# NVlabs/STEP

Measured on NVIDIA H100. Metric: clips/sec (T=32,224x224) STEP max_iter=3, higher is better.
Workload: dtype f16

## Files before the change

### step_b200/_lib.py

```python
import ctypes
import os

import torch

HERE = os.path.dirname(os.path.abspath(__file__))
LIB_PATH = os.path.join(HERE, "libstep_b200.so")

F32, F16 = 0, 1
EXT_NONE, EXT_PREDICT, EXT_EXTRAPOLATE, EXT_MEAN = 0, 1, 2, 3
A_AUTO, A_LINEAR, A_BOX, A_IM2COL, A_HALO, A_BEST, A_SIMT = 0, 1, 2, 3, 4, 5, 9

_lib = None

c_int, c_float, c_void_p, c_size_t = ctypes.c_int, ctypes.c_float, ctypes.c_void_p, ctypes.c_size_t


class ConvParams(ctypes.Structure):
    _fields_ = [(n, c_int) for n in
                ("dtype", "N", "T", "H", "W", "Cin", "in_ld", "Cout", "out_ld", "out_coff", "KT", "KH", "KW",
                 "ST", "SH", "SW", "PT", "PH", "PW", "OT", "OH", "OW", "relu", "w_ld")] + \
               [("x", c_void_p), ("w", c_void_p), ("scale", c_void_p), ("shift", c_void_p),
                ("residual", c_void_p), ("res_ld", c_int), ("res_coff", c_int), ("y", c_void_p),
                ("a_mode", c_int), ("n_splits", c_int), ("split", c_int * 2), ("y_extra", c_void_p * 2),
                ("ld_extra", c_int * 2), ("coff_extra", c_int * 2), ("zero_cin_last_kt", c_int)]
# ... 37 lines not shown
        "step_clip_to_s2d_f16": ([P, I, I, I, I, I, P, I, S], c_int),
        "step_nhwc_to_nchw_f32": ([P, I, I, I, I, I, P, S], c_int),
        "step_nchw_to_nhwc": ([P, I, I, I, P, I, I, S], c_int),
        "step_conv3d_fwd": ([ctypes.POINTER(ConvParams), S], c_int),
        "step_maxpool3d_fwd": ([P, I] + [I] * 21 + [P, I, S], c_int),
        "step_mean_mid": ([P, I, I, I, I, I, I, P, I, S], c_int),
        "step_mean_mid_strided": ([P, I, I, I, I, I, I, ctypes.c_longlong, P, I, S], c_int),
        "step_linear_small_n_workspace_bytes": ([I, I, I], c_size_t),
        "step_linear_small_n": ([P, I, I, I, I, P, P, I, P, I, I, I, P, P, c_size_t, S], c_int),
        "step_head_regress": ([P, I, I, I, I, I, P, P, I, I, I, I, P, P, P, P, c_size_t, S], c_int),
        "step_bottleneck_exit_f16": ([P, ctypes.c_longlong, P, P, ctypes.c_longlong, P, P, I, P, ctypes.c_longlong, P, ctypes.c_longlong,
                                     ctypes.c_longlong, I, I, I, S], c_int),
        "step_head_losses_f32": ([P, P, P, P, P, P, I, I, I, I, I, Fl, Fl, P, P, P, P, P, P, P, P, P, S], c_int),
        "step_cls_loss_f32": ([P, P, I, I, P, P, P, S], c_int),
        "step_roi_align_bwd_nhwc": ([P, I, I, P, I, Fl, I, I, I, I, I, I, I, P, I, S], c_int),
        "step_roi_align_bwd_slice_workspace_bytes": ([I, I, I, I, I, I], c_size_t),
        "step_roi_align_bwd_slice_nhwc": ([P, I, I, P, I, Fl, I, I, I, I, I, I, I, I, I, I, P, I, P, c_size_t, S], c_int),
        "step_ctx_grad_reduce_f32": ([P, I, P, I, I, I, I, I, I, P, S], c_int),
        "step_linear_small_n_bwd": ([P, I, I, I, I, P, P, I, P, I, P, P, S], c_int),
        "step_conv1x1_wgrad_workspace_bytes": ([I, I, I], c_size_t),
        "step_conv1x1_wgrad_f16": ([P, I, P, I, I, I, I, Fl, P, I, I, P, c_size_t, S], c_int),
        "step_conv_wgrad_workspace_bytes": ([I, I, I, I], c_size_t),
        "step_conv_wgrad_f16": ([P, I, P, I, I, I, I, I, I, I, I, I, I, I, I, I, Fl, P, I, I, P, c_size_t, S], c_int),
        "step_act_bwd_f16": ([P, I, P, I, P, I, ctypes.c_longlong, I, P, I, P, I, S], c_int),
        "step_colsum_f16": ([P, I, ctypes.c_longlong, I, Fl, P, P, S], c_int),
        "step_mean_mid_bwd": ([P, I, I, I, I, Fl, P, I, S], c_int),
        "step_f32_accum_f16": ([P, ctypes.c_longlong, I, Fl, P, I, S], c_int),
        "step_maxpool3d_bwd_f16": ([P, I, P, I] + [I] * 20 + [P, I, P, S], c_int),
        "step_multi_tensor_chunk": ([], c_int),
        "step_multi_tensor_nonfinite_f32": ([P, I, P, I, P, S], c_int),
        "step_multi_tensor_adam_f32": ([P, I, P, I, S], c_int),
        "step_multi_tensor_sgd_f32": ([P, I, P, I, S], c_int),
        "step_debug_tma_tile": ([ctypes.POINTER(ConvParams), I, I, I, I, I, P, P, P, S], c_int),
    }
    for name, (argtypes, restype) in sigs.items():
        fn = getattr(lib, name)
        fn.argtypes = argtypes
        fn.restype = restype
    return sigs


def lib():
    global _lib
    if _lib is None:
        if not os.path.exists(LIB_PATH):
            raise RuntimeError("step_b200: %s not found -- run `python -m step_b200.build` (there is no "
                               "CPU / PyTorch fallback for the hot path)" % LIB_PATH)
        l = ctypes.CDLL(LIB_PATH)
        _declare(l)
        _lib = l
    return _lib


def exported_symbols():
    return sorted(_declare(lib()).keys())


def check(rc):
    if rc != 0:
        raise RuntimeError("step_b200 [%d]: %s" % (rc, lib().step_last_error().decode("utf-8", "replace")))


def stream(device=None):
    return c_void_p(torch.cuda.current_stream(device).cuda_stream)


# ... 35 lines not shown
```

### step_b200/csrc/conv_umma.cu

```cuda
#include <cuda.h>
#include <stdlib.h>
#include <string.h>

#include "common.cuh"
#include "umma_ptx.cuh"

namespace step {

enum { A_LINEAR = 1, A_BOX = 2, A_IM2COL = 3 };

constexpr int kBM = 128;
constexpr int kMaxBN = 256;
constexpr int kStages = 8;
constexpr int kThreads = 384;
constexpr int kConsumers = 256;
constexpr int kBookBytes = 2 * kStages * 8 + 2 * kMaxBN * 4;
constexpr int kProducerRegs = 40, kConsumerRegs = 232;

#define STEP_CONV_TILES(X)                                                                                         \
  X(64, 32) X(64, 64) X(64, 128) X(64, 144) X(64, 152) X(64, 176) X(64, 192) X(64, 208) X(64, 224) X(64, 256)      \
  X(32, 64) X(32, 128) X(32, 144) X(32, 152) X(32, 160) X(32, 208) X(32, 224)                                      \
  X(16, 64)

__host__ __device__ constexpr int staging_pitch(int BN) { return ((BN / 8 + 1) | 1) * 16; }

struct ConvGeom {
  int mode;
  int taps, KT, KH, KW, PT, PH, PW;
  int kblocks_per_tap;
  int BN, n_tiles;
  int n_stages;
  int n_splits, split[2], ld_extra[2], coff_extra[2];
  __half* y_extra[2];
  int Cout, out_ld, out_coff, res_ld, res_coff, relu;
  int OT, OH, OW, Nimg;
  long long M;
  int bw, bh, bt, tiles_w, tiles_h, tiles_t;
  int a_bytes;
};

__device__ __forceinline__ long long tile_row_pixel(const ConvGeom& g, int m_tile, int row) {
  if (g.mode == A_BOX) {
    int r = m_tile;
    const int bw0 = (r % g.tiles_w) * g.bw; r /= g.tiles_w;
    const int bh0 = (r % g.tiles_h) * g.bh; r /= g.tiles_h;
    const int bt0 = (r % g.tiles_t) * g.bt; const int bn = r / g.tiles_t;
    const int dw = row % g.bw, rr = row / g.bw;
    const int dh = rr % g.bh, dt = rr / g.bh;
    const int ow = bw0 + dw, oh = bh0 + dh, ot = bt0 + dt;
    if (dt < g.bt && ow < g.OW && oh < g.OH && ot < g.OT) return (((long long)bn * g.OT + ot) * g.OH + oh) * g.OW + ow;
    return -1;
  }
  const long long m = (long long)m_tile * kBM + row;
  return m < g.M ? m : -1;
}

template <int BK, int BN>
__global__ void __launch_bounds__(kThreads, 1)
conv_umma_kernel(const __grid_constant__ CUtensorMap map_a, const __grid_constant__ CUtensorMap map_b, ConvGeom g,
                 const float* __restrict__ scale, const float* __restrict__ shift, const __half* __restrict__ residual,
                 __half* __restrict__ y) {
  static_assert(BN % 8 == 0 && BN <= kMaxBN, "wgmma N is a multiple of 8, at most 256");
  constexpr bool kRealloc = BN > 128;
  constexpr int kABytes = kBM * BK * 2;
  constexpr int kBBytes = BN * BK * 2;
  extern __shared__ __align__(1024) uint8_t smem_raw[];
  uint64_t* full_bar = (uint64_t*)smem_raw;
  uint64_t* empty_bar = full_bar + kStages;
  float* s_scale = (float*)(empty_bar + kStages);
  float* s_shift = s_scale + kMaxBN;
  uint8_t* smem = (uint8_t*)(((uintptr_t)smem_raw + kBookBytes + 1023) & ~(uintptr_t)1023);
  uint8_t* sA = smem;
  uint8_t* sB = smem + g.n_stages * kABytes;

  const int warp = threadIdx.x >> 5, lane = threadIdx.x & 31;
  const int m_tile = blockIdx.x / g.n_tiles, n_tile = blockIdx.x - m_tile * g.n_tiles;
  const int n0 = n_tile * BN;
  const int num_kb = g.taps * g.kblocks_per_tap;

  if (threadIdx.x == 0) {
    asm volatile("prefetch.tensormap [%0];" ::"l"(&map_a) : "memory");
    asm volatile("prefetch.tensormap [%0];" ::"l"(&map_b) : "memory");
    for (int s = 0; s < kStages; ++s) { mbar_init(&full_bar[s], 1); mbar_init(&empty_bar[s], 2); }
    fence_barrier_init();
  }
  if (threadIdx.x < 128) {
    for (int i = threadIdx.x; i < BN; i += 128) {
      const int c = n0 + i;
      s_scale[i] = (scale && c < g.Cout) ? scale[c] : 1.0f;
      s_shift[i] = (shift && c < g.Cout) ? shift[c] : 0.0f;
    }
  }
  __syncthreads();
  pdl_wait();
  pdl_launch_dependents();

  if (warp < 4) {
    if constexpr (kRealloc) setmaxnreg_dec<kProducerRegs>();
    if (warp == 0 && elect_one()) {
      long long m0 = (long long)m_tile * kBM;
      int bn = 0, bt0 = 0, bh0 = 0, bw0 = 0;
      if (g.mode == A_BOX) {
        int r = m_tile;
        bw0 = (r % g.tiles_w) * g.bw; r /= g.tiles_w;
        bh0 = (r % g.tiles_h) * g.bh; r /= g.tiles_h;
        bt0 = (r % g.tiles_t) * g.bt; bn = r / g.tiles_t;
      }
      int iw = 0, ih = 0, it = 0, in_ = 0;
      if (g.mode == A_IM2COL) {
        long long r = m0;
        iw = (int)(r % g.OW); r /= g.OW;
        ih = (int)(r % g.OH); r /= g.OH;
        it = (int)(r % g.OT); in_ = (int)(r / g.OT);
        iw -= g.PW; ih -= g.PH; it -= g.PT;
      }
      const uint32_t tx_bytes = (uint32_t)(g.a_bytes + kBBytes);
      int stage = 0; uint32_t phase = 0;
      int kw = 0, kh = 0, kt = 0;
      for (int tap = 0; tap < g.taps; ++tap) {
        for (int kc = 0; kc < g.kblocks_per_tap; ++kc) {
          mbar_wait(&empty_bar[stage], phase ^ 1);
          mbar_expect_tx(&full_bar[stage], tx_bytes);
          const int c0 = kc * BK;
          uint8_t* a_dst = sA + stage * kABytes;
          if (g.mode == A_LINEAR) {
            tma_load_2d(&map_a, &full_bar[stage], a_dst, c0, (int)m0);
          } else if (g.mode == A_BOX) {
            tma_load_5d(&map_a, &full_bar[stage], a_dst, c0, bw0 + kw - g.PW, bh0 + kh - g.PH, bt0 + kt - g.PT, bn);
          } else {
            tma_load_im2col_5d(&map_a, &full_bar[stage], a_dst, c0, iw, ih, it, in_, (uint16_t)kw, (uint16_t)kh, (uint16_t)kt);
          }
          tma_load_3d(&map_b, &full_bar[stage], sB + stage * kBBytes, c0, tap, n0);
          if (++stage == g.n_stages) { stage = 0; phase ^= 1; }
        }
        if (++kw == g.KW) { kw = 0; if (++kh == g.KH) { kh = 0; ++kt; } }
      }
    }
  } else {
    if constexpr (kRealloc) setmaxnreg_inc<kConsumerRegs>();
    const int wg = (warp >> 2) - 1;
    const int ct = threadIdx.x - 128;
    const uint64_t hi = desc_hi_kmajor<BK>();
    const uint64_t a_lo0 = desc_lo(sA + wg * 64 * BK * 2), b_lo0 = desc_lo(sB);
    float acc[BN / 2];
#pragma unroll
    for (int i = 0; i < BN / 2; ++i) acc[i] = 0.0f;
    int stage = 0, prev = -1; uint32_t phase = 0;
    for (int kb = 0; kb < num_kb; ++kb) {
      mbar_wait(&full_bar[stage], phase);
      const uint64_t a_lo = a_lo0 + (uint64_t)(stage * (kABytes >> 4)), b_lo = b_lo0 + (uint64_t)(stage * (kBBytes >> 4));
      wg_fence();
#pragma unroll
      for (int k = 0; k < BK / 16; ++k)
        wgmma_f16<BN>(acc, hi | (a_lo + 2 * k), hi | (b_lo + 2 * k), 1u);
      wg_commit();
      wg_wait<1>();
      if (prev >= 0 && ct % 128 == 0) mbar_arrive(&empty_bar[prev]);
      prev = stage;
      if (++stage == g.n_stages) { stage = 0; phase ^= 1; }
    }
    wg_wait<0>();
    named_sync(1, kConsumers);
    constexpr int pitch = staging_pitch(BN);
    const int wrow = wg * 64 + (warp & 3) * 16 + (lane >> 2);
#pragma unroll
    for (int i = 0; i < 2; ++i) {
      const int row = wrow + 8 * i;
      const long long pix = residual ? tile_row_pixel(g, m_tile, row) : -1;
      const __half* rrow = pix >= 0 ? residual + (size_t)pix * g.res_ld + g.res_coff + n0 : nullptr;
      uint8_t* srow = smem + (size_t)row * pitch;
#pragma unroll
      for (int j = 0; j < BN / 8; ++j) {
        const int col = 8 * j + 2 * (lane & 3);
        float f0 = fmaf(acc[4 * j + 2 * i], s_scale[col], s_shift[col]);
        float f1 = fmaf(acc[4 * j + 2 * i + 1], s_scale[col + 1], s_shift[col + 1]);
        if (rrow && n0 + col < g.Cout) {
          const float2 rf = __half22float2(*reinterpret_cast<const __half2*>(rrow + col));
          f0 += rf.x; f1 += rf.y;
        }
        if (g.relu) { f0 = fmaxf(f0, 0.0f); f1 = fmaxf(f1, 0.0f); }
        *reinterpret_cast<__half2*>(srow + col * 2) = __floats2half2_rn(f0, f1);
      }
    }
    named_sync(1, kConsumers);
    constexpr int cpr = BN / 8;
    for (int i = ct; i < kBM * cpr; i += kConsumers) {
      const int rr = i / cpr, ch = i - rr * cpr;
      const int col = n0 + ch * 8;
      if (col >= g.Cout) continue;
      const long long rp = tile_row_pixel(g, m_tile, rr);
      if (rp < 0) continue;
      const uint4 val = *reinterpret_cast<const uint4*>(smem + (size_t)rr * pitch + ch * 16);
      __half* dst = y + (size_t)rp * g.out_ld + g.out_coff + col;
      if (g.n_splits > 0 && col >= g.split[0]) {
        const int d = (g.n_splits > 1 && col >= g.split[1]) ? 1 : 0;
        dst = g.y_extra[d] + (size_t)rp * g.ld_extra[d] + g.coff_extra[d] + (col - g.split[d]);
      }
      *reinterpret_cast<uint4*>(dst) = val;
    }
  }
}

template <int BK>
__global__ void __launch_bounds__(32) tma_dump_kernel(const __grid_constant__ CUtensorMap map_a, ConvGeom g, int m_tile,
                                                      int kt, int kh, int kw, int c0, uint8_t* __restrict__ out) {
  constexpr int kABytes = kBM * BK * 2;
  extern __shared__ __align__(1024) uint8_t smem_raw[];
  uint8_t* smem = (uint8_t*)(((uintptr_t)smem_raw + 1023) & ~(uintptr_t)1023);
  __shared__ uint64_t bar;
  for (int i = threadIdx.x; i < kABytes / 4; i += 32) ((uint32_t*)smem)[i] = 0xFFFFFFFFu;
  if (threadIdx.x == 0) { mbar_init(&bar, 1); fence_barrier_init(); }
  fence_proxy_async();
  __syncwarp();
  if (threadIdx.x == 0) {
    long long m0 = (long long)m_tile * kBM;
    mbar_expect_tx(&bar, (uint32_t)g.a_bytes);
    if (g.mode == A_LINEAR) {
      tma_load_2d(&map_a, &bar, smem, c0, (int)m0);
    } else if (g.mode == A_BOX) {
      int r = m_tile;
      int bw0 = (r % g.tiles_w) * g.bw; r /= g.tiles_w;
      int bh0 = (r % g.tiles_h) * g.bh; r /= g.tiles_h;
      int bt0 = (r % g.tiles_t) * g.bt; int bn = r / g.tiles_t;
      tma_load_5d(&map_a, &bar, smem, c0, bw0 + kw - g.PW, bh0 + kh - g.PH, bt0 + kt - g.PT, bn);
    } else {
      long long r = m0;
      int iw = (int)(r % g.OW); r /= g.OW;
      int ih = (int)(r % g.OH); r /= g.OH;
      int it = (int)(r % g.OT); int in_ = (int)(r / g.OT);
      tma_load_im2col_5d(&map_a, &bar, smem, c0, iw - g.PW, ih - g.PH, it - g.PT, in_, (uint16_t)kw, (uint16_t)kh, (uint16_t)kt);
    }
// ... 158 lines not shown
                             (cuuint64_t)p->H * p->W * p->in_ld * 2, (cuuint64_t)p->T * p->H * p->W * p->in_ld * 2};
    if (mode == A_BOX) {
      pick_box(p->OW, p->OH, p->OT, &g.bw, &g.bh, &g.bt);
      g.tiles_w = (p->OW + g.bw - 1) / g.bw; g.tiles_h = (p->OH + g.bh - 1) / g.bh; g.tiles_t = (p->OT + g.bt - 1) / g.bt;
      cuuint32_t box[5] = {(cuuint32_t)BK, (cuuint32_t)g.bw, (cuuint32_t)g.bh, (cuuint32_t)g.bt, 1};
      cr = g_encode_tiled(&pl->map_a, CU_TENSOR_MAP_DATA_TYPE_FLOAT16, 5, (void*)p->x, dims, strides, box, ones,
                          CU_TENSOR_MAP_INTERLEAVE_NONE, swizzle_for(BK), CU_TENSOR_MAP_L2_PROMOTION_L2_128B,
                          CU_TENSOR_MAP_FLOAT_OOB_FILL_NONE);
      m_tiles = (long long)p->N * g.tiles_t * g.tiles_h * g.tiles_w;
      g.a_bytes = g.bw * g.bh * g.bt * BK * 2;
    } else {
      const int ph_t = p->OT - p->T + p->KT - 1 - p->PT, ph_h = p->OH - p->H + p->KH - 1 - p->PH,
                ph_w = p->OW - p->W + p->KW - 1 - p->PW;
      int lower[3] = {-p->PW, -p->PH, -p->PT};
      int upper[3] = {ph_w - (p->KW - 1), ph_h - (p->KH - 1), ph_t - (p->KT - 1)};
      for (int i = 0; i < 3; ++i)
        STEP_CHECK_ARG(lower[i] >= -16 && lower[i] <= 15 && upper[i] >= -16 && upper[i] <= 15, "conv3d(f16): im2col corner range");
      cr = g_encode_im2col(&pl->map_a, CU_TENSOR_MAP_DATA_TYPE_FLOAT16, 5, (void*)p->x, dims, strides, lower, upper,
                           (cuuint32_t)BK, (cuuint32_t)kBM, ones, CU_TENSOR_MAP_INTERLEAVE_NONE, swizzle_for(BK),
                           CU_TENSOR_MAP_L2_PROMOTION_L2_128B, CU_TENSOR_MAP_FLOAT_OOB_FILL_NONE);
      int drv = 0;
      cudaDriverGetVersion(&drv);
      if (cr == CUDA_SUCCESS && drv <= 13010 &&
          (size_t)p->N * p->T * p->H * p->W * p->in_ld * 2 < 131072)
        reinterpret_cast<uint64_t*>(&pl->map_a)[1] &= ~(1ULL << 21);
      m_tiles = (g.M + kBM - 1) / kBM;
      g.a_bytes = kBM * BK * 2;
    }
  }
  if (cr != CUDA_SUCCESS) return fail(STEP_E_DRIVER, "conv3d(f16): tensor map (A, mode %d) encode failed: CUresult %d", mode, (int)cr);
  {
    cuuint64_t dims[3] = {(cuuint64_t)p->Cin, (cuuint64_t)taps, (cuuint64_t)p->Cout};
    cuuint64_t strides[2] = {(cuuint64_t)p->w_ld * 2, (cuuint64_t)taps * p->w_ld * 2};
    cuuint32_t box[3] = {(cuuint32_t)BK, 1, (cuuint32_t)g.BN};
    cr = g_encode_tiled(&pl->map_b, CU_TENSOR_MAP_DATA_TYPE_FLOAT16, 3, (void*)p->w, dims, strides, box, ones,
                        CU_TENSOR_MAP_INTERLEAVE_NONE, swizzle_for(BK), CU_TENSOR_MAP_L2_PROMOTION_L2_256B,
                        CU_TENSOR_MAP_FLOAT_OOB_FILL_NONE);
    if (cr != CUDA_SUCCESS) return fail(STEP_E_DRIVER, "conv3d(f16): tensor map (B) encode failed: CUresult %d", (int)cr);
  }
  STEP_CHECK_ARG(m_tiles * g.n_tiles < (1LL << 31), "conv3d(f16): grid too large");
  pl->grid = dim3((unsigned)(m_tiles * g.n_tiles));
  const long per_stage = (long)kBM * BK * 2 + (long)g.BN * BK * 2;
  const long fixed = kBookBytes + 1024;
  const long out_tile = (long)kBM * staging_pitch(g.BN);
  int st = (int)((113L * 1024 - fixed) / per_stage);
  if (st > kStages) st = kStages;
  bool two = false;
  if (st >= 4) {
    const long area = st * per_stage;
    if (int rc = two_ctas_fit(pl->tile, (size_t)(fixed + (area > out_tile ? area : out_tile)), &two)) return rc;
  }
  if (!two) st = (int)((227L * 1024 - fixed) / per_stage);
  g.n_stages = st > kStages ? kStages : st;
  STEP_CHECK_ARG(g.n_stages >= 2, "conv3d(f16): tile does not fit shared memory");
  const long stage_area = g.n_stages * per_stage;
  pl->smem_bytes = (size_t)(fixed + (stage_area > out_tile ? stage_area : out_tile));
  return 0;
}

int conv3d_umma_launch(const step_conv_params* p, step_stream_t stream) {
  ConvPlan pl;
  if (int rc = build_plan(p, &pl)) return rc;
  const ConvTile& t = kTiles[pl.tile];
  if (first_use_on_device(g_attr_seen[pl.tile])) {
    cudaError_t e = cudaFuncSetAttribute(t.kernel, cudaFuncAttributeMaxDynamicSharedMemorySize, 227 * 1024);
    if (e != cudaSuccess) return fail((int)e, "conv3d(f16): smem attribute: %s", cudaGetErrorString(e));
  }
  cudaStream_t s = cu(stream);
  cudaLaunchConfig_t cfg = {};
  cudaLaunchAttribute attr[1];
  cfg.gridDim = pl.grid; cfg.blockDim = dim3(kThreads); cfg.dynamicSmemBytes = pl.smem_bytes; cfg.stream = s;
  if (pdl_enabled()) {
    attr[0].id = cudaLaunchAttributeProgrammaticStreamSerialization;
    attr[0].val.programmaticStreamSerializationAllowed = 1;
    cfg.attrs = attr; cfg.numAttrs = 1;
  }
  cudaError_t le = cudaLaunchKernelEx(&cfg, t.kernel, pl.map_a, pl.map_b, pl.g, p->scale, p->shift,
                                      (const __half*)p->residual, (__half*)p->y);
  if (le != cudaSuccess) { cudaGetLastError(); return fail((int)le, "conv_umma_kernel launch: %s", cudaGetErrorString(le)); }
  STEP_LAUNCH_CHECK("conv_umma_kernel");
  return 0;
}

}

using namespace step;

extern "C" int step_debug_tma_tile(const step_conv_params* p, int m_tile, int kt, int kh, int kw, int c0, void* out,
                                   int* bk_out, int* box_out , step_stream_t stream) {
  ConvPlan pl;
  if (int rc = build_plan(p, &pl)) return rc;
  if (bk_out) *bk_out = pl.BK;
  if (box_out) { box_out[0] = pl.g.bw; box_out[1] = pl.g.bh; box_out[2] = pl.g.bt; }
  size_t smem = 1024 + (size_t)kBM * pl.BK * 2;
  if (pl.BK == 64) tma_dump_kernel<64><<<1, 32, smem, cu(stream)>>>(pl.map_a, pl.g, m_tile, kt, kh, kw, c0, (uint8_t*)out);
  else if (pl.BK == 32) tma_dump_kernel<32><<<1, 32, smem, cu(stream)>>>(pl.map_a, pl.g, m_tile, kt, kh, kw, c0, (uint8_t*)out);
  else tma_dump_kernel<16><<<1, 32, smem, cu(stream)>>>(pl.map_a, pl.g, m_tile, kt, kh, kw, c0, (uint8_t*)out);
  STEP_LAUNCH_CHECK("tma_dump_kernel");
  return 0;
}
```

### step_b200/csrc/umma_ptx.cuh

```cuda
#pragma once
#include <cuda.h>
#include <cuda_fp16.h>
#include <stdint.h>

namespace step {

__device__ __forceinline__ uint32_t smem_u32(const void* p) { return (uint32_t)__cvta_generic_to_shared(p); }

__device__ __forceinline__ void mbar_init(uint64_t* bar, uint32_t count) {
  asm volatile("mbarrier.init.shared::cta.b64 [%0], %1;" ::"r"(smem_u32(bar)), "r"(count));
}
__device__ __forceinline__ void mbar_expect_tx(uint64_t* bar, uint32_t bytes) {
  asm volatile("mbarrier.arrive.expect_tx.shared::cta.b64 _, [%0], %1;" ::"r"(smem_u32(bar)), "r"(bytes) : "memory");
}
__device__ __forceinline__ void mbar_arrive(uint64_t* bar) {
  asm volatile("mbarrier.arrive.shared::cta.b64 _, [%0];" ::"r"(smem_u32(bar)) : "memory");
}
__device__ __forceinline__ void mbar_wait(uint64_t* bar, uint32_t parity) {
  asm volatile(
      "{\n\t.reg .pred p;\n\t"
      "WAIT_LOOP:\n\t"
      "mbarrier.try_wait.parity.shared::cta.b64 p, [%0], %1;\n\t"
      "@p bra.uni WAIT_DONE;\n\t"
      "bra.uni WAIT_LOOP;\n\t"
// ... 22 lines not shown
               ::"r"(smem_u32(dst)), "l"(map), "r"(smem_u32(bar)), "r"(c), "r"(w), "r"(h), "r"(d), "r"(n), "h"(ow), "h"(oh), "h"(od) : "memory");
}
__device__ __forceinline__ void tma_store_2d(const CUtensorMap* map, const void* src, int c0, int c1) {
  asm volatile("cp.async.bulk.tensor.2d.global.shared::cta.bulk_group [%0, {%2, %3}], [%1];"
               ::"l"(map), "r"(smem_u32(src)), "r"(c0), "r"(c1) : "memory");
}
__device__ __forceinline__ void bulk_commit() { asm volatile("cp.async.bulk.commit_group;" ::: "memory"); }
template <int N>
__device__ __forceinline__ void bulk_wait_read() { asm volatile("cp.async.bulk.wait_group.read %0;" ::"n"(N) : "memory"); }

template <int BK>
__device__ __forceinline__ uint64_t desc_hi_kmajor() {
  constexpr uint64_t sw = BK == 64 ? 1 : (BK == 32 ? 2 : 3);
  return (1ULL << 16) | ((uint64_t)((8 * BK * 2) >> 4) << 32) | (sw << 62);
}
__device__ __forceinline__ uint64_t desc_lo(const void* p) { return (uint64_t)((smem_u32(p) & 0x3FFFF) >> 4); }

__device__ __forceinline__ void wg_fence() { asm volatile("wgmma.fence.sync.aligned;" ::: "memory"); }
__device__ __forceinline__ void wg_commit() { asm volatile("wgmma.commit_group.sync.aligned;" ::: "memory"); }
template <int N>
__device__ __forceinline__ void wg_wait() { asm volatile("wgmma.wait_group.sync.aligned %0;" ::"n"(N) : "memory"); }

template <int N>
__device__ __forceinline__ void wgmma_f16(float* d, uint64_t da, uint64_t db, uint32_t accumulate);

#define STEP_D4(i) "+f"(d[4 * (i)]), "+f"(d[4 * (i) + 1]), "+f"(d[4 * (i) + 2]), "+f"(d[4 * (i) + 3])
#define STEP_WGMMA_F16(N, IA, IB, IC, REGS, ...)                                                                        \
  template <>                                                                                                          \
  __device__ __forceinline__ void wgmma_f16<N>(float* d, uint64_t da, uint64_t db, uint32_t accumulate) {              \
    asm volatile("{\n\t.reg .pred p;\n\tsetp.ne.b32 p, %" #IC ", 0;\n\t"                                              \
                 "wgmma.mma_async.sync.aligned.m64n" #N "k16.f32.f16.f16 {" REGS "}, %" #IA ", %" #IB ", p, 1, 1, 0, 0;\n\t}" \
                 : __VA_ARGS__ : "l"(da), "l"(db), "r"(accumulate));                                                    \
  }
STEP_WGMMA_F16(32, 16, 17, 18,
               "%0, %1, %2, %3, %4, %5, %6, %7, %8, %9, %10, %11, %12, %13, %14, %15",
               STEP_D4(0), STEP_D4(1), STEP_D4(2), STEP_D4(3))
STEP_WGMMA_F16(64, 32, 33, 34,
               "%0, %1, %2, %3, %4, %5, %6, %7, %8, %9, %10, %11, %12, %13, %14, %15, %16, %17, %18, %19, %20, %21, %22, "
               "%23, %24, %25, %26, %27, %28, %29, %30, %31",
               STEP_D4(0), STEP_D4(1), STEP_D4(2), STEP_D4(3), STEP_D4(4), STEP_D4(5), STEP_D4(6), STEP_D4(7))
STEP_WGMMA_F16(128, 64, 65, 66,
               "%0, %1, %2, %3, %4, %5, %6, %7, %8, %9, %10, %11, %12, %13, %14, %15, %16, %17, %18, %19, %20, %21, %22, "
               "%23, %24, %25, %26, %27, %28, %29, %30, %31, %32, %33, %34, %35, %36, %37, %38, %39, %40, %41, %42, %43, "
               "%44, %45, %46, %47, %48, %49, %50, %51, %52, %53, %54, %55, %56, %57, %58, %59, %60, %61, %62, %63",
               STEP_D4(0), STEP_D4(1), STEP_D4(2), STEP_D4(3), STEP_D4(4), STEP_D4(5), STEP_D4(6), STEP_D4(7),
               STEP_D4(8), STEP_D4(9), STEP_D4(10), STEP_D4(11), STEP_D4(12), STEP_D4(13), STEP_D4(14), STEP_D4(15))
STEP_WGMMA_F16(144, 72, 73, 74,
               "%0, %1, %2, %3, %4, %5, %6, %7, %8, %9, %10, %11, %12, %13, %14, %15, %16, %17, %18, %19, %20, %21, %22, "
               "%23, %24, %25, %26, %27, %28, %29, %30, %31, %32, %33, %34, %35, %36, %37, %38, %39, %40, %41, %42, %43, "
               "%44, %45, %46, %47, %48, %49, %50, %51, %52, %53, %54, %55, %56, %57, %58, %59, %60, %61, %62, %63, %64, "
               "%65, %66, %67, %68, %69, %70, %71",
               STEP_D4(0), STEP_D4(1), STEP_D4(2), STEP_D4(3), STEP_D4(4), STEP_D4(5), STEP_D4(6), STEP_D4(7),
               STEP_D4(8), STEP_D4(9), STEP_D4(10), STEP_D4(11), STEP_D4(12), STEP_D4(13), STEP_D4(14), STEP_D4(15),
               STEP_D4(16), STEP_D4(17))
STEP_WGMMA_F16(152, 76, 77, 78,
               "%0, %1, %2, %3, %4, %5, %6, %7, %8, %9, %10, %11, %12, %13, %14, %15, %16, %17, %18, %19, %20, %21, %22, "
               "%23, %24, %25, %26, %27, %28, %29, %30, %31, %32, %33, %34, %35, %36, %37, %38, %39, %40, %41, %42, %43, "
               "%44, %45, %46, %47, %48, %49, %50, %51, %52, %53, %54, %55, %56, %57, %58, %59, %60, %61, %62, %63, %64, "
               "%65, %66, %67, %68, %69, %70, %71, %72, %73, %74, %75",
               STEP_D4(0), STEP_D4(1), STEP_D4(2), STEP_D4(3), STEP_D4(4), STEP_D4(5), STEP_D4(6), STEP_D4(7),
               STEP_D4(8), STEP_D4(9), STEP_D4(10), STEP_D4(11), STEP_D4(12), STEP_D4(13), STEP_D4(14), STEP_D4(15),
               STEP_D4(16), STEP_D4(17), STEP_D4(18))
STEP_WGMMA_F16(160, 80, 81, 82,
               "%0, %1, %2, %3, %4, %5, %6, %7, %8, %9, %10, %11, %12, %13, %14, %15, %16, %17, %18, %19, %20, %21, %22, "
               "%23, %24, %25, %26, %27, %28, %29, %30, %31, %32, %33, %34, %35, %36, %37, %38, %39, %40, %41, %42, %43, "
               "%44, %45, %46, %47, %48, %49, %50, %51, %52, %53, %54, %55, %56, %57, %58, %59, %60, %61, %62, %63, %64, "
               "%65, %66, %67, %68, %69, %70, %71, %72, %73, %74, %75, %76, %77, %78, %79",
               STEP_D4(0), STEP_D4(1), STEP_D4(2), STEP_D4(3), STEP_D4(4), STEP_D4(5), STEP_D4(6), STEP_D4(7),
               STEP_D4(8), STEP_D4(9), STEP_D4(10), STEP_D4(11), STEP_D4(12), STEP_D4(13), STEP_D4(14), STEP_D4(15),
               STEP_D4(16), STEP_D4(17), STEP_D4(18), STEP_D4(19))
STEP_WGMMA_F16(176, 88, 89, 90,
               "%0, %1, %2, %3, %4, %5, %6, %7, %8, %9, %10, %11, %12, %13, %14, %15, %16, %17, %18, %19, %20, %21, %22, "
               "%23, %24, %25, %26, %27, %28, %29, %30, %31, %32, %33, %34, %35, %36, %37, %38, %39, %40, %41, %42, %43, "
// ... 96 lines not shown
```

Before: 1099.

## Make wgmma conv kernel persistent with half-width tail tiles and per-group epilogue

Turns the wgmma conv kernel into a persistent kernel that loops over work units with grid capped at SM slots. To cut wave-quantization tail waste, the remainder tiles are split into two half-N units using narrower wgmma shapes, and B is loaded in two half boxes. The epilogue now runs per warpgroup through a dedicated chunked staging buffer with per-group scale/shift, so each group syncs independently and smem is no longer aliased with pipeline stages. This costs extra shared memory, which may reduce pipeline stages, and adds more template code and register pressure. It also adds a debug plan query entry point.

Measured after the change: 1112 (median of 6 runs). +1.1%, better.

```diff
diff --git a/step_b200/_lib.py b/step_b200/_lib.py
--- a/step_b200/_lib.py
+++ b/step_b200/_lib.py
@@ -93,6 +93,7 @@
         "step_multi_tensor_adam_f32": ([P, I, P, I, S], c_int),
         "step_multi_tensor_sgd_f32": ([P, I, P, I, S], c_int),
         "step_debug_tma_tile": ([ctypes.POINTER(ConvParams), I, I, I, I, I, P, P, P, S], c_int),
+        "step_debug_conv_plan": ([ctypes.POINTER(ConvParams), P], c_int),
     }
     for name, (argtypes, restype) in sigs.items():
         fn = getattr(lib, name)
diff --git a/step_b200/csrc/conv_umma.cu b/step_b200/csrc/conv_umma.cu
--- a/step_b200/csrc/conv_umma.cu
+++ b/step_b200/csrc/conv_umma.cu
@@ -13,8 +13,7 @@
 constexpr int kMaxBN = 256;
 constexpr int kStages = 8;
 constexpr int kThreads = 384;
-constexpr int kConsumers = 256;
-constexpr int kBookBytes = 2 * kStages * 8 + 2 * kMaxBN * 4;
+constexpr int kBookBytes = 2 * kStages * 8 + 2 * 2 * kMaxBN * 4;
 constexpr int kProducerRegs = 40, kConsumerRegs = 232;
 
 #define STEP_CONV_TILES(X)                                                                                         \
@@ -22,7 +21,11 @@
   X(32, 64) X(32, 128) X(32, 144) X(32, 152) X(32, 160) X(32, 208) X(32, 224)                                      \
   X(16, 64)
 
-__host__ __device__ constexpr int staging_pitch(int BN) { return ((BN / 8 + 1) | 1) * 16; }
+__host__ __device__ constexpr int staging_pitch(int cols) { return ((cols / 8 + 1) | 1) * 16; }
+constexpr int kChunk = 64;
+constexpr int kGroupStaging = 64 * staging_pitch(kChunk);
+constexpr int kStagingBytes = 2 * kGroupStaging;
+__host__ __device__ constexpr bool halves_ok(int BN) { return BN % 16 == 0; }
 
 struct ConvGeom {
   int mode;
@@ -30,6 +33,7 @@
   int kblocks_per_tap;
   int BN, n_tiles;
   int n_stages;
+  int units, full_units;
   int n_splits, split[2], ld_extra[2], coff_extra[2];
   __half* y_extra[2];
   int Cout, out_ld, out_coff, res_ld, res_coff, relu;
@@ -55,27 +59,58 @@
   return m < g.M ? m : -1;
 }
 
+template <int BN>
+__device__ __forceinline__ void unit_tile(const ConvGeom& g, int u, int* m_tile, int* n0, bool* half) {
+  int t = u, h = 0;
+  *half = u >= g.full_units;
+  if (*half) { t = g.full_units + ((u - g.full_units) >> 1); h = (u - g.full_units) & 1; }
+  *m_tile = t / g.n_tiles;
+  *n0 = (t - *m_tile * g.n_tiles) * BN + h * (BN / 2);
+}
+
+template <int BK, int BN, int N>
+__device__ __forceinline__ void mma_unit(float* acc, uint64_t hi, uint64_t a_lo0, uint64_t b_lo0, int num_kb, int n_stages,
+                                         uint64_t* full_bar, uint64_t* empty_bar, bool leader, int& stage, uint32_t& phase) {
+  constexpr int kABytes = kBM * BK * 2;
+  constexpr int kBBytes = BN * BK * 2;
+  int prev = -1;
+  for (int kb = 0; kb < num_kb; ++kb) {
+    mbar_wait(&full_bar[stage], phase);
+    const uint64_t a_lo = a_lo0 + (uint64_t)(stage * (kABytes >> 4)), b_lo = b_lo0 + (uint64_t)(stage * (kBBytes >> 4));
+    wg_fence();
+#pragma unroll
+    for (int k = 0; k < BK / 16; ++k)
+      wgmma_f16<N>(acc, hi | (a_lo + 2 * k), hi | (b_lo + 2 * k), 1u);
+    wg_commit();
+    wg_wait<1>();
+    if (prev >= 0 && leader) mbar_arrive(&empty_bar[prev]);
+    prev = stage;
+    if (++stage == n_stages) { stage = 0; phase ^= 1; }
+  }
+  wg_wait<0>();
+  if (leader) mbar_arrive(&empty_bar[prev]);
+}
+
 template <int BK, int BN>
-__global__ void __launch_bounds__(kThreads, 1)
+__global__ void __launch_bounds__(kThreads, BN <= 64 ? 2 : 1)
 conv_umma_kernel(const __grid_constant__ CUtensorMap map_a, const __grid_constant__ CUtensorMap map_b, ConvGeom g,
                  const float* __restrict__ scale, const float* __restrict__ shift, const __half* __restrict__ residual,
                  __half* __restrict__ y) {
   static_assert(BN % 8 == 0 && BN <= kMaxBN, "wgmma N is a multiple of 8, at most 256");
   constexpr bool kRealloc = BN > 128;
+  constexpr bool kHalves = halves_ok(BN);
   constexpr int kABytes = kBM * BK * 2;
   constexpr int kBBytes = BN * BK * 2;
   extern __shared__ __align__(1024) uint8_t smem_raw[];
   uint64_t* full_bar = (uint64_t*)smem_raw;
   uint64_t* empty_bar = full_bar + kStages;
-  float* s_scale = (float*)(empty_bar + kStages);
-  float* s_shift = s_scale + kMaxBN;
+  float* epi_const = (float*)(empty_bar + kStages);
   uint8_t* smem = (uint8_t*)(((uintptr_t)smem_raw + kBookBytes + 1023) & ~(uintptr_t)1023);
   uint8_t* sA = smem;
   uint8_t* sB = smem + g.n_stages * kABytes;
+  uint8_t* staging = sB + g.n_stages * kBBytes;
 
   const int warp = threadIdx.x >> 5, lane = threadIdx.x & 31;
-  const int m_tile = blockIdx.x / g.n_tiles, n_tile = blockIdx.x - m_tile * g.n_tiles;
-  const int n0 = n_tile * BN;
   const int num_kb = g.taps * g.kblocks_per_tap;
 
   if (threadIdx.x == 0) {
@@ -84,13 +119,6 @@
     for (int s = 0; s < kStages; ++s) { mbar_init(&full_bar[s], 1); mbar_init(&empty_bar[s], 2); }
     fence_barrier_init();
   }
-  if (threadIdx.x < 128) {
-    for (int i = threadIdx.x; i < BN; i += 128) {
-      const int c = n0 + i;
-      s_scale[i] = (scale && c < g.Cout) ? scale[c] : 1.0f;
-      s_shift[i] = (shift && c < g.Cout) ? shift[c] : 0.0f;
-    }
-  }
   __syncthreads();
   pdl_wait();
   pdl_launch_dependents();
@@ -98,105 +126,129 @@
   if (warp < 4) {
     if constexpr (kRealloc) setmaxnreg_dec<kProducerRegs>();
     if (warp == 0 && elect_one()) {
-      long long m0 = (long long)m_tile * kBM;
-      int bn = 0, bt0 = 0, bh0 = 0, bw0 = 0;
-      if (g.mode == A_BOX) {
-        int r = m_tile;
-        bw0 = (r % g.tiles_w) * g.bw; r /= g.tiles_w;
-        bh0 = (r % g.tiles_h) * g.bh; r /= g.tiles_h;
-        bt0 = (r % g.tiles_t) * g.bt; bn = r / g.tiles_t;
-      }
-      int iw = 0, ih = 0, it = 0, in_ = 0;
-      if (g.mode == A_IM2COL) {
-        long long r = m0;
-        iw = (int)(r % g.OW); r /= g.OW;
-        ih = (int)(r % g.OH); r /= g.OH;
-        it = (int)(r % g.OT); in_ = (int)(r / g.OT);
-        iw -= g.PW; ih -= g.PH; it -= g.PT;
-      }
-      const uint32_t tx_bytes = (uint32_t)(g.a_bytes + kBBytes);
       int stage = 0; uint32_t phase = 0;
-      int kw = 0, kh = 0, kt = 0;
-      for (int tap = 0; tap < g.taps; ++tap) {
-        for (int kc = 0; kc < g.kblocks_per_tap; ++kc) {
-          mbar_wait(&empty_bar[stage], phase ^ 1);
-          mbar_expect_tx(&full_bar[stage], tx_bytes);
-          const int c0 = kc * BK;
-          uint8_t* a_dst = sA + stage * kABytes;
-          if (g.mode == A_LINEAR) {
-            tma_load_2d(&map_a, &full_bar[stage], a_dst, c0, (int)m0);
-          } else if (g.mode == A_BOX) {
-            tma_load_5d(&map_a, &full_bar[stage], a_dst, c0, bw0 + kw - g.PW, bh0 + kh - g.PH, bt0 + kt - g.PT, bn);
-          } else {
-            tma_load_im2col_5d(&map_a, &full_bar[stage], a_dst, c0, iw, ih, it, in_, (uint16_t)kw, (uint16_t)kh, (uint16_t)kt);
+      for (int u = blockIdx.x; u < g.units; u += gridDim.x) {
+        int m_tile, n0; bool half;
+        unit_tile<BN>(g, u, &m_tile, &n0, &half);
+        const long long m0 = (long long)m_tile * kBM;
+        int bn = 0, bt0 = 0, bh0 = 0, bw0 = 0;
+        if (g.mode == A_BOX) {
+          int r = m_tile;
+          bw0 = (r % g.tiles_w) * g.bw; r /= g.tiles_w;
+          bh0 = (r % g.tiles_h) * g.bh; r /= g.tiles_h;
+          bt0 = (r % g.tiles_t) * g.bt; bn = r / g.tiles_t;
+        }
+        int iw = 0, ih = 0, it = 0, in_ = 0;
+        if (g.mode == A_IM2COL) {
+          long long r = m0;
+          iw = (int)(r % g.OW); r /= g.OW;
+          ih = (int)(r % g.OH); r /= g.OH;
+          it = (int)(r % g.OT); in_ = (int)(r / g.OT);
+          iw -= g.PW; ih -= g.PH; it -= g.PT;
+        }
+        const uint32_t tx_bytes = (uint32_t)(g.a_bytes + (half ? kBBytes / 2 : kBBytes));
+        int kw = 0, kh = 0, kt = 0;
+        for (int tap = 0; tap < g.taps; ++tap) {
+          for (int kc = 0; kc < g.kblocks_per_tap; ++kc) {
+            mbar_wait(&empty_bar[stage], phase ^ 1);
+            mbar_expect_tx(&full_bar[stage], tx_bytes);
+            const int c0 = kc * BK;
+            uint8_t* a_dst = sA + stage * kABytes;
+            if (g.mode == A_LINEAR) {
+              tma_load_2d(&map_a, &full_bar[stage], a_dst, c0, (int)m0);
+            } else if (g.mode == A_BOX) {
+              tma_load_5d(&map_a, &full_bar[stage], a_dst, c0, bw0 + kw - g.PW, bh0 + kh - g.PH, bt0 + kt - g.PT, bn);
+            } else {
+              tma_load_im2col_5d(&map_a, &full_bar[stage], a_dst, c0, iw, ih, it, in_, (uint16_t)kw, (uint16_t)kh, (uint16_t)kt);
+            }
+            uint8_t* b_dst = sB + stage * kBBytes;
+            tma_load_3d(&map_b, &full_bar[stage], b_dst, c0, tap, n0);
+            if (kHalves && !half) tma_load_3d(&map_b, &full_bar[stage], b_dst + kBBytes / 2, c0, tap, n0 + BN / 2);
+            if (++stage == g.n_stages) { stage = 0; phase ^= 1; }
           }
-          tma_load_3d(&map_b, &full_bar[stage], sB + stage * kBBytes, c0, tap, n0);
-          if (++stage == g.n_stages) { stage = 0; phase ^= 1; }
+          if (++kw == g.KW) { kw = 0; if (++kh == g.KH) { kh = 0; ++kt; } }
         }
-        if (++kw == g.KW) { kw = 0; if (++kh == g.KH) { kh = 0; ++kt; } }
       }
     }
   } else {
     if constexpr (kRealloc) setmaxnreg_inc<kConsumerRegs>();
     const int wg = (warp >> 2) - 1;
-    const int ct = threadIdx.x - 128;
+    const bool leader = (threadIdx.x & 127) == 0;
     const uint64_t hi = desc_hi_kmajor<BK>();
     const uint64_t a_lo0 = desc_lo(sA + wg * 64 * BK * 2), b_lo0 = desc_lo(sB);
+    constexpr int pitch = staging_pitch(kChunk);
+    uint8_t* wstage = staging + wg * kGroupStaging;
+    float* s_scale = epi_const + wg * 2 * kMaxBN;
+    float* s_shift = s_scale + kMaxBN;
+    const int wt = threadIdx.x & 127;
+    const int lrow = (warp & 3) * 16 + (lane >> 2);
+    const int q = lane & 3;
     float acc[BN / 2];
-#pragma unroll
-    for (int i = 0; i < BN / 2; ++i) acc[i] = 0.0f;
-    int stage = 0, prev = -1; uint32_t phase = 0;
-    for (int kb = 0; kb < num_kb; ++kb) {
-      mbar_wait(&full_bar[stage], phase);
-      const uint64_t a_lo = a_lo0 + (uint64_t)(stage * (kABytes >> 4)), b_lo = b_lo0 + (uint64_t)(stage * (kBBytes >> 4));
-      wg_fence();
-#pragma unroll
-      for (int k = 0; k < BK / 16; ++k)
-        wgmma_f16<BN>(acc, hi | (a_lo + 2 * k), hi | (b_lo + 2 * k), 1u);
-      wg_commit();
-      wg_wait<1>();
-      if (prev >= 0 && ct % 128 == 0) mbar_arrive(&empty_bar[prev]);
-      prev = stage;
-      if (++stage == g.n_stages) { stage = 0; phase ^= 1; }
-    }
-    wg_wait<0>();
-    named_sync(1, kConsumers);
-    constexpr int pitch = staging_pitch(BN);
-    const int wrow = wg * 64 + (warp & 3) * 16 + (lane >> 2);
-#pragma unroll
-    for (int i = 0; i < 2; ++i) {
-      const int row = wrow + 8 * i;
-      const long long pix = residual ? tile_row_pixel(g, m_tile, row) : -1;
-      const __half* rrow = pix >= 0 ? residual + (size_t)pix * g.res_ld + g.res_coff + n0 : nullptr;
-      uint8_t* srow = smem + (size_t)row * pitch;
-#pragma unroll
-      for (int j = 0; j < BN / 8; ++j) {
-        const int col = 8 * j + 2 * (lane & 3);
-        float f0 = fmaf(acc[4 * j + 2 * i], s_scale[col], s_shift[col]);
-        float f1 = fmaf(acc[4 * j + 2 * i + 1], s_scale[col + 1], s_shift[col + 1]);
-        if (rrow && n0 + col < g.Cout) {
-          const float2 rf = __half22float2(*reinterpret_cast<const __half2*>(rrow + col));
-          f0 += rf.x; f1 += rf.y;
+    int stage = 0; uint32_t phase = 0;
+    for (int u = blockIdx.x; u < g.units; u += gridDim.x) {
+      int m_tile, n0; bool half;
+      unit_tile<BN>(g, u, &m_tile, &n0, &half);
+      const int ncols = half ? BN / 2 : BN;
+      for (int i = wt; i < ncols; i += 128) {
+        const int c = n0 + i;
+        s_scale[i] = (scale && c < g.Cout) ? scale[c] : 1.0f;
+        s_shift[i] = (shift && c < g.Cout) ? shift[c] : 0.0f;
+      }
+#pragma unroll
+      for (int i = 0; i < BN / 2; ++i) acc[i] = 0.0f;
+      if constexpr (kHalves) {
+        if (half) mma_unit<BK, BN, BN / 2>(acc, hi, a_lo0, b_lo0, num_kb, g.n_stages, full_bar, empty_bar, leader, stage, phase);
+        else mma_unit<BK, BN, BN>(acc, hi, a_lo0, b_lo0, num_kb, g.n_stages, full_bar, empty_bar, leader, stage, phase);
+      } else {
+        mma_unit<BK, BN, BN>(acc, hi, a_lo0, b_lo0, num_kb, g.n_stages, full_bar, empty_bar, leader, stage, phase);
+      }
+      const __half* rrow[2];
+#pragma unroll
+      for (int i = 0; i < 2; ++i) {
+        const long long pix = residual ? tile_row_pixel(g, m_tile, wg * 64 + lrow + 8 * i) : -1;
+        rrow[i] = pix >= 0 ? residual + (size_t)pix * g.res_ld + g.res_coff + n0 : nullptr;
+      }
+      long long opix[4];
+#pragma unroll
+      for (int k = 0; k < 4; ++k) opix[k] = tile_row_pixel(g, m_tile, wg * 64 + (wt >> 3) + 16 * k);
+      named_sync(1 + wg, 128);
+#pragma unroll
+      for (int c = 0; c < (BN + kChunk - 1) / kChunk; ++c) {
+        if (c * kChunk >= ncols) break;
+#pragma unroll
+        for (int jj = 0; jj < kChunk / 8; ++jj) {
+          const int j = c * (kChunk / 8) + jj;
+          if (j >= BN / 8 || 8 * j >= ncols) break;
+          const int col = 8 * j + 2 * q;
+#pragma unroll
+          for (int i = 0; i < 2; ++i) {
+            float f0 = fmaf(acc[4 * j + 2 * i], s_scale[col], s_shift[col]);
+            float f1 = fmaf(acc[4 * j + 2 * i + 1], s_scale[col + 1], s_shift[col + 1]);
+            if (rrow[i] && n0 + col < g.Cout) {
+              const float2 rf = __half22float2(*reinterpret_cast<const __half2*>(rrow[i] + col));
+              f0 += rf.x; f1 += rf.y;
+            }
+            if (g.relu) { f0 = fmaxf(f0, 0.0f); f1 = fmaxf(f1, 0.0f); }
+            *reinterpret_cast<__half2*>(wstage + (lrow + 8 * i) * pitch + (col - c * kChunk) * 2) = __floats2half2_rn(f0, f1);
+          }
         }
-        if (g.relu) { f0 = fmaxf(f0, 0.0f); f1 = fmaxf(f1, 0.0f); }
-        *reinterpret_cast<__half2*>(srow + col * 2) = __floats2half2_rn(f0, f1);
+        named_sync(1 + wg, 128);
+        const int ccol = c * kChunk + 8 * (wt & 7), col = n0 + ccol;
+        if (ccol < ncols && col < g.Cout) {
+#pragma unroll
+          for (int k = 0; k < 4; ++k) {
+            if (opix[k] < 0) continue;
+            const uint4 val = *reinterpret_cast<const uint4*>(wstage + ((wt >> 3) + 16 * k) * pitch + (wt & 7) * 16);
+            __half* dst = y + (size_t)opix[k] * g.out_ld + g.out_coff + col;
+            if (g.n_splits > 0 && col >= g.split[0]) {
+              const int d = (g.n_splits > 1 && col >= g.split[1]) ? 1 : 0;
+              dst = g.y_extra[d] + (size_t)opix[k] * g.ld_extra[d] + g.coff_extra[d] + (col - g.split[d]);
+            }
+            *reinterpret_cast<uint4*>(dst) = val;
+          }
+        }
+        named_sync(1 + wg, 128);
       }
-    }
-    named_sync(1, kConsumers);
-    constexpr int cpr = BN / 8;
-    for (int i = ct; i < kBM * cpr; i += kConsumers) {
-      const int rr = i / cpr, ch = i - rr * cpr;
-      const int col = n0 + ch * 8;
-      if (col >= g.Cout) continue;
-      const long long rp = tile_row_pixel(g, m_tile, rr);
-      if (rp < 0) continue;
-      const uint4 val = *reinterpret_cast<const uint4*>(smem + (size_t)rr * pitch + ch * 16);
-      __half* dst = y + (size_t)rp * g.out_ld + g.out_coff + col;
-      if (g.n_splits > 0 && col >= g.split[0]) {
-        const int d = (g.n_splits > 1 && col >= g.split[1]) ? 1 : 0;
-        dst = g.y_extra[d] + (size_t)rp * g.ld_extra[d] + g.coff_extra[d] + (col - g.split[d]);
-      }
-      *reinterpret_cast<uint4*>(dst) = val;
     }
   }
 }
@@ -421,29 +473,35 @@
   {
     cuuint64_t dims[3] = {(cuuint64_t)p->Cin, (cuuint64_t)taps, (cuuint64_t)p->Cout};
     cuuint64_t strides[2] = {(cuuint64_t)p->w_ld * 2, (cuuint64_t)taps * p->w_ld * 2};
-    cuuint32_t box[3] = {(cuuint32_t)BK, 1, (cuuint32_t)g.BN};
+    cuuint32_t box[3] = {(cuuint32_t)BK, 1, (cuuint32_t)(halves_ok(g.BN) ? g.BN / 2 : g.BN)};
     cr = g_encode_tiled(&pl->map_b, CU_TENSOR_MAP_DATA_TYPE_FLOAT16, 3, (void*)p->w, dims, strides, box, ones,
                         CU_TENSOR_MAP_INTERLEAVE_NONE, swizzle_for(BK), CU_TENSOR_MAP_L2_PROMOTION_L2_256B,
                         CU_TENSOR_MAP_FLOAT_OOB_FILL_NONE);
     if (cr != CUDA_SUCCESS) return fail(STEP_E_DRIVER, "conv3d(f16): tensor map (B) encode failed: CUresult %d", (int)cr);
   }
-  STEP_CHECK_ARG(m_tiles * g.n_tiles < (1LL << 31), "conv3d(f16): grid too large");
-  pl->grid = dim3((unsigned)(m_tiles * g.n_tiles));
+  const long long tiles = m_tiles * g.n_tiles;
+  STEP_CHECK_ARG(2 * tiles < (1LL << 31), "conv3d(f16): grid too large");
   const long per_stage = (long)kBM * BK * 2 + (long)g.BN * BK * 2;
-  const long fixed = kBookBytes + 1024;
-  const long out_tile = (long)kBM * staging_pitch(g.BN);
+  const long fixed = kBookBytes + 1024 + kStagingBytes;
   int st = (int)((113L * 1024 - fixed) / per_stage);
   if (st > kStages) st = kStages;
   bool two = false;
-  if (st >= 4) {
-    const long area = st * per_stage;
-    if (int rc = two_ctas_fit(pl->tile, (size_t)(fixed + (area > out_tile ? area : out_tile)), &two)) return rc;
-  }
+  if (st >= 4)
+    if (int rc = two_ctas_fit(pl->tile, (size_t)(fixed + st * per_stage), &two)) return rc;
   if (!two) st = (int)((227L * 1024 - fixed) / per_stage);
   g.n_stages = st > kStages ? kStages : st;
   STEP_CHECK_ARG(g.n_stages >= 2, "conv3d(f16): tile does not fit shared memory");
-  const long stage_area = g.n_stages * per_stage;
-  pl->smem_bytes = (size_t)(fixed + (stage_area > out_tile ? stage_area : out_tile));
+  pl->smem_bytes = (size_t)(fixed + g.n_stages * per_stage);
+  int dev = 0, sms = 0;
+  cudaError_t e = cudaGetDevice(&dev);
+  if (e == cudaSuccess) e = cudaDeviceGetAttribute(&sms, cudaDevAttrMultiProcessorCount, dev);
+  if (e != cudaSuccess) { cudaGetLastError(); return fail((int)e, "conv3d(f16): SM count: %s", cudaGetErrorString(e)); }
+  const long long slots = (long long)sms * (two ? 2 : 1);
+  const long long rem = tiles % slots;
+  const long long split = (halves_ok(g.BN) && 2 * rem <= slots) ? rem : 0;
+  g.full_units = (int)(tiles - split);
+  g.units = (int)(tiles + split);
+  pl->grid = dim3((unsigned)(g.units < slots ? g.units : slots));
   return 0;
 }
 
@@ -488,3 +546,11 @@
   STEP_LAUNCH_CHECK("tma_dump_kernel");
   return 0;
 }
+
+extern "C" int step_debug_conv_plan(const step_conv_params* p, int* out ) {
+  ConvPlan pl;
+  if (int rc = build_plan(p, &pl)) return rc;
+  const int v[6] = {pl.BK, pl.g.BN, pl.g.n_stages, (int)pl.grid.x, pl.g.units, pl.g.full_units};
+  for (int i = 0; i < 6; ++i) out[i] = v[i];
+  return 0;
+}
diff --git a/step_b200/csrc/umma_ptx.cuh b/step_b200/csrc/umma_ptx.cuh
--- a/step_b200/csrc/umma_ptx.cuh
+++ b/step_b200/csrc/umma_ptx.cuh
@@ -78,6 +78,9 @@
                  "wgmma.mma_async.sync.aligned.m64n" #N "k16.f32.f16.f16 {" REGS "}, %" #IA ", %" #IB ", p, 1, 1, 0, 0;\n\t}" \
                  : __VA_ARGS__ : "l"(da), "l"(db), "r"(accumulate));                                                    \
   }
+STEP_WGMMA_F16(16, 8, 9, 10,
+               "%0, %1, %2, %3, %4, %5, %6, %7",
+               STEP_D4(0), STEP_D4(1))
 STEP_WGMMA_F16(32, 16, 17, 18,
                "%0, %1, %2, %3, %4, %5, %6, %7, %8, %9, %10, %11, %12, %13, %14, %15",
                STEP_D4(0), STEP_D4(1), STEP_D4(2), STEP_D4(3))
@@ -85,6 +88,39 @@
                "%0, %1, %2, %3, %4, %5, %6, %7, %8, %9, %10, %11, %12, %13, %14, %15, %16, %17, %18, %19, %20, %21, %22, "
                "%23, %24, %25, %26, %27, %28, %29, %30, %31",
                STEP_D4(0), STEP_D4(1), STEP_D4(2), STEP_D4(3), STEP_D4(4), STEP_D4(5), STEP_D4(6), STEP_D4(7))
+STEP_WGMMA_F16(72, 36, 37, 38,
+               "%0, %1, %2, %3, %4, %5, %6, %7, %8, %9, %10, %11, %12, %13, %14, %15, %16, %17, %18, %19, %20, %21, %22, "
+               "%23, %24, %25, %26, %27, %28, %29, %30, %31, %32, %33, %34, %35",
+               STEP_D4(0), STEP_D4(1), STEP_D4(2), STEP_D4(3), STEP_D4(4), STEP_D4(5), STEP_D4(6), STEP_D4(7),
+               STEP_D4(8))
+STEP_WGMMA_F16(80, 40, 41, 42,
+               "%0, %1, %2, %3, %4, %5, %6, %7, %8, %9, %10, %11, %12, %13, %14, %15, %16, %17, %18, %19, %20, %21, %22, "
+               "%23, %24, %25, %26, %27, %28, %29, %30, %31, %32, %33, %34, %35, %36, %37, %38, %39",
+               STEP_D4(0), STEP_D4(1), STEP_D4(2), STEP_D4(3), STEP_D4(4), STEP_D4(5), STEP_D4(6), STEP_D4(7),
+               STEP_D4(8), STEP_D4(9))
+STEP_WGMMA_F16(88, 44, 45, 46,
+               "%0, %1, %2, %3, %4, %5, %6, %7, %8, %9, %10, %11, %12, %13, %14, %15, %16, %17, %18, %19, %20, %21, %22, "
+               "%23, %24, %25, %26, %27, %28, %29, %30, %31, %32, %33, %34, %35, %36, %37, %38, %39, %40, %41, %42, %43",
+               STEP_D4(0), STEP_D4(1), STEP_D4(2), STEP_D4(3), STEP_D4(4), STEP_D4(5), STEP_D4(6), STEP_D4(7),
+               STEP_D4(8), STEP_D4(9), STEP_D4(10))
+STEP_WGMMA_F16(96, 48, 49, 50,
+               "%0, %1, %2, %3, %4, %5, %6, %7, %8, %9, %10, %11, %12, %13, %14, %15, %16, %17, %18, %19, %20, %21, %22, "
+               "%23, %24, %25, %26, %27, %28, %29, %30, %31, %32, %33, %34, %35, %36, %37, %38, %39, %40, %41, %42, %43, "
+               "%44, %45, %46, %47",
+               STEP_D4(0), STEP_D4(1), STEP_D4(2), STEP_D4(3), STEP_D4(4), STEP_D4(5), STEP_D4(6), STEP_D4(7),
+               STEP_D4(8), STEP_D4(9), STEP_D4(10), STEP_D4(11))
+STEP_WGMMA_F16(104, 52, 53, 54,
+               "%0, %1, %2, %3, %4, %5, %6, %7, %8, %9, %10, %11, %12, %13, %14, %15, %16, %17, %18, %19, %20, %21, %22, "
+               "%23, %24, %25, %26, %27, %28, %29, %30, %31, %32, %33, %34, %35, %36, %37, %38, %39, %40, %41, %42, %43, "
+               "%44, %45, %46, %47, %48, %49, %50, %51",
+               STEP_D4(0), STEP_D4(1), STEP_D4(2), STEP_D4(3), STEP_D4(4), STEP_D4(5), STEP_D4(6), STEP_D4(7),
+               STEP_D4(8), STEP_D4(9), STEP_D4(10), STEP_D4(11), STEP_D4(12))
+STEP_WGMMA_F16(112, 56, 57, 58,
+               "%0, %1, %2, %3, %4, %5, %6, %7, %8, %9, %10, %11, %12, %13, %14, %15, %16, %17, %18, %19, %20, %21, %22, "
+               "%23, %24, %25, %26, %27, %28, %29, %30, %31, %32, %33, %34, %35, %36, %37, %38, %39, %40, %41, %42, %43, "
+               "%44, %45, %46, %47, %48, %49, %50, %51, %52, %53, %54, %55",
+               STEP_D4(0), STEP_D4(1), STEP_D4(2), STEP_D4(3), STEP_D4(4), STEP_D4(5), STEP_D4(6), STEP_D4(7),
+               STEP_D4(8), STEP_D4(9), STEP_D4(10), STEP_D4(11), STEP_D4(12), STEP_D4(13))
 STEP_WGMMA_F16(128, 64, 65, 66,
                "%0, %1, %2, %3, %4, %5, %6, %7, %8, %9, %10, %11, %12, %13, %14, %15, %16, %17, %18, %19, %20, %21, %22, "
                "%23, %24, %25, %26, %27, %28, %29, %30, %31, %32, %33, %34, %35, %36, %37, %38, %39, %40, %41, %42, %43, "
```
